# WGLab/DeepMod

Hardware: AMD Instinct MI355X
Metric: base-positions/sec (whole node), E. coli 5mC wd21/f7 BiLSTM (higher is better)
Workload: dtype f16x3

## Files before the change

### deepmod_amd/csrc/kern_f16q0.hip

```cpp
#include "kernels.h"
#include <utility>
#include "lstm_common.hip.inc"
#include "lstm_f16q.hip.inc"

static_assert(lstm16q::TILE_M == dmk::TILE_M, "work item size");

namespace {
inline void fill(lstmc::Params& p, const dmk::F16Args& a) {
    p.wpack = a.wpack;
    p.wpack_i8 = a.wpack;
    p.hpack = a.hpack;
    p.bout0 = p.bout1 = 0.0f;
    p.x = a.x;
    p.xstride = a.xstride;
    p.widx = a.widx;
    p.n = a.n;
    p.ntiles = a.ntiles;
    p.plogit = a.plogit;
    p.len_scale = std::ldexp(1.0f, -a.len_shift);
    p.len_mul = std::ldexp(1.0f, a.len_shift);
    p.range_flag = a.range_flag;
    for (int k = 0; k < 24; ++k) p.i8s[k] = a.i8s ? a.i8s[k] : 0.0f;
}
}
// ... 65 lines not shown
                                    d8[1] = (signed char)std::max(-127.0f, std::min(127.0f, ql));
                                }
                            }
                        }
                }
                for (int mrec = 0; mrec < (l == 0 ? 2 : 1); ++mrec) {
                    _Float16* dst = reinterpret_cast<_Float16*>(P.w.data() + off);
                    off += MIX_BYTES;
                    for (int rh = 0; rh < 2; ++rh)
                        for (int lane = 0; lane < 64; ++lane) {
                            const int m = lane & 15, g = lane >> 4;
                            const int unit = 8 * S + 4 * rh + m / 4, gate = m % 4;
                            _Float16 slot[8];
                            for (int j = 0; j < 8; ++j) slot[j] = (_Float16)0.0f;
                            if (unit < HID) {
                                const int gc = gate * 100 + unit;
                                _Float16 hi, lo;
                                if (mrec == 0) {
                                    split(wval(kin + 96 + g, gc, 1.0f), hi, lo);
                                    slot[0] = hi; slot[1] = lo; slot[2] = hi;
                                    split(wval(l == 0 ? g : 96 + g, gc, 1.0f), hi, lo);
                                    slot[3] = hi; slot[4] = lo; slot[5] = hi;
                                    if (g == 0) {
                                        split(wval(-2, gc, 1.0f), hi, lo);
                                        slot[6] = hi; slot[7] = lo;
                                    }
                                } else {
                                    split(g < 3 ? wval(4 + g, gc, 1.0f) : wval(NFEAT - 1, gc, len_mul), hi, lo);
                                    slot[0] = hi; slot[1] = lo; slot[2] = hi; slot[3] = lo;
                                }
                            }
                            for (int j = 0; j < 8; ++j) dst[(size_t(rh) * 64 + lane) * 8 + j] = slot[j];
                        }
                }
            }
        }
    }
    return P;
}


hipError_t f16q_prepare(int mm) {
    if (mm == 1) return f16q1_prepare();
    return hipFuncSetAttribute(reinterpret_cast<const void*>(lstm16q::bilstm_f16q_kernel<0>), hipFuncAttributeMaxDynamicSharedMemorySize, int(lstm16q::LDS_BYTES));
}
void f16q_launch(int mm, const F16Args& a, int grid, hipStream_t stream) {
    if (mm == 1) return f16q1_launch(a, grid, stream);
    lstmc::Params p;
    fill(p, a);
    hipLaunchKernelGGL(lstm16q::bilstm_f16q_kernel<0>, dim3(grid), dim3(lstm16q::THREADS), lstm16q::LDS_BYTES, stream, p);
}

}
```

### deepmod_amd/csrc/kern_f16q1.hip

```cpp
#include "kernels.h"
#include <utility>
#include "lstm_common.hip.inc"
#include "lstm_f16q.hip.inc"

namespace {
inline void fill(lstmc::Params& p, const dmk::F16Args& a) {
    p.wpack = a.wpack;
    p.wpack_i8 = a.wpack;
    p.hpack = a.hpack;
    p.bout0 = p.bout1 = 0.0f;
    p.x = a.x;
    p.xstride = a.xstride;
    p.widx = a.widx;
    p.n = a.n;
    p.ntiles = a.ntiles;
    p.plogit = a.plogit;
    p.len_scale = std::ldexp(1.0f, -a.len_shift);
    p.len_mul = std::ldexp(1.0f, a.len_shift);
    p.range_flag = a.range_flag;
    for (int k = 0; k < 24; ++k) p.i8s[k] = a.i8s ? a.i8s[k] : 0.0f;
}
}

namespace dmk {

hipError_t f16q1_prepare() {
    return hipFuncSetAttribute(reinterpret_cast<const void*>(lstm16q::bilstm_f16q_kernel<1>), hipFuncAttributeMaxDynamicSharedMemorySize, int(lstm16q::LDS_BYTES_I8));
}
void f16q1_launch(const F16Args& a, int grid, hipStream_t stream) {
    lstmc::Params p;
    fill(p, a);
    hipLaunchKernelGGL(lstm16q::bilstm_f16q_kernel<1>, dim3(grid), dim3(lstm16q::THREADS), lstm16q::LDS_BYTES_I8, stream, p);
}

}
```

### deepmod_amd/csrc/kernels.h

```cpp
#pragma once
#include <hip/hip_runtime.h>

#if defined(DM16Q_ABL_NOCELL) || defined(DM16Q_ABL_NODMA) || defined(DM16Q_ABL_MIX1) || defined(DM16Q_ABL_I8T) || defined(DM16Q_ABL_NOBAR) || defined(DM16Q_ABL_NOVMWAIT) || defined(DM16Q_AINIT) || defined(DM16Q_DEBUG_NOP) ||           \
    defined(DM16Q_NOCHUNK) || defined(DM16Q_NOPN) || defined(DM16Q_LOPACK) || defined(DM16Q_PRE) || defined(DM16Q_SNAKE) || defined(DM16Q_TRANS_COST) ||                     \
    defined(DM16S_ABL_2PROD) || defined(DM16S_ABL_B64) || defined(DM16S_ABL_LO_ONLY) || defined(DM16S_ABL_MFMA16) ||                              \
    defined(DM16S_ABL_MFMA16_PAD) || defined(DM16S_ABL_NOBAR) || defined(DM16S_ABL_NOCELL) || defined(DM16S_ABL_NODMA) ||                          \
    defined(DM16S_ABL_NOLDSA) || defined(DM16S_ADIST) || defined(DM16S_ALO_TRUNC) || defined(DM16S_PRE) || defined(DM_ABL_NOBAR) ||                \
    defined(DM_ABL_NODMA) || defined(DM_ABL_NOEPI) || defined(DM_ABL_NOSEQ) || defined(DM_TIMING) || defined(DM_TRACE) || defined(DM_TRACE2) ||   \
    defined(DM_WLO_TRUNC_ENV) || defined(DM_WLO_TRUNC_DEFAULT) || defined(DM_WITH_F16X3_ROLES) || defined(DM16R_DMA_M) ||                         \
    defined(DM_F16X3_SHAPE_DEFAULT) || defined(DM_WAVES) || defined(DM_MT) || defined(DM_WITH_F16S)
#define DM_ANY_EXPERIMENT_SWITCH 1
#ifndef DM_EXPERIMENT
#error "an ablation / experiment macro is defined without -DDM_EXPERIMENT: timing-only kernels must not be built into the product by a stray -D"
#endif
#else
#define DM_ANY_EXPERIMENT_SWITCH 0
#endif


#if defined(DM_WITH_F16X3_ROLES) && !defined(DM_WITH_F16S)
#error "the roles experiment lives in the translation unit of the 32x32x16 kernels: build it with -DDM_WITH_F16S as well"
#endif

#include <algorithm>
#include <cmath>
#include <cstdint>
#include <cstdlib>
#include <cstring>
#include <vector>

#include "../../include/deepmod_hip.h"

#ifndef DM_F16X3_SHAPE_DEFAULT
#define DM_F16X3_SHAPE_DEFAULT 16
#endif

namespace dmk {

constexpr int TILE_M = 128;

inline float gate_scale(int gc) { return (gc >= 100 && gc < 200) ? 2.8853900817779268f : -1.4426950408889634f; }


struct Packed32 {
    std::vector<float> w, b, h;
    float bout[2];
};

struct Packed16 {
    std::vector<unsigned char> w;
    float max_abs = 0.0f;
    bool finite = true;
    int len_shift = 0;
};

inline int choose_len_shift(const float* flat) {
    float m = 0.0f;
// ... 61 lines not shown
```

### deepmod_amd/csrc/lstm_f16q.hip.inc

```
#ifndef DM16Q_TRANS_COST
#define DM16Q_TRANS_COST 2
#endif
namespace lstm16q {

using lstmc::floatx2;
using lstmc::floatx4;
using lstmc::halfx2;
using lstmc::halfx8;
using lstmc::uintx4;
using lstmc::Params;
using lstmc::ex2;
using lstmc::rcp;
using lstmc::min60;
using lstmc::split_pack;
using lstmc::static_for;
using lstmc::as_h8;

constexpr int HID = 100, NFEAT = 7, WIN = 21, LIVE = 11;
constexpr int NTILE = 13;
constexpr int WAVES = 4, THREADS = 64 * WAVES, TILE_M = 32 * WAVES;
constexpr int KS_L0 = 4, KS_L12 = 7;
constexpr int REC_BYTES = 4096;
constexpr int MIX_BYTES = 2048;
constexpr int TILE_BYTES_L0 = (KS_L0 - 1) * REC_BYTES + 2 * MIX_BYTES, TILE_BYTES_L12 = (KS_L12 - 1) * REC_BYTES + MIX_BYTES;
constexpr int SLOT_BYTES = TILE_BYTES_L12;
constexpr int NSLOT = 2;
constexpr int C2_WAVE_BYTES = NTILE * 1024;
constexpr int C2_LAYER_BYTES = WAVES * C2_WAVE_BYTES;
constexpr size_t LDS_BYTES = size_t(NSLOT) * SLOT_BYTES + C2_LAYER_BYTES;
constexpr size_t LDS_BYTES_I8 = LDS_BYTES + C2_LAYER_BYTES;
constexpr size_t WEIGHT_BYTES_DIR = size_t(NTILE) * (TILE_BYTES_L0 + 2 * TILE_BYTES_L12);
constexpr size_t WEIGHT_BYTES = 2 * WEIGHT_BYTES_DIR;

using lstmc::intx4;
using lstmc::I8_MAGIC;
using lstmc::I8_HI_SCALE;
using lstmc::I8_LO_SCALE;
struct CellPipe {
    float ef[4], ei[4], ej[4], eo[4], t0[4], t1[4];
    unsigned hi01, hi23, lo01, lo23, i01, i23;
    floatx2 fold[2];
    floatx2 kmagic, khi, klo;
    static constexpr int NM = 14;
    template <int PRE, int FMT>
    __device__ static constexpr int nops(int M) {
        constexpr int n[9] = {12, 12, 12, 12, 8, 4, 4, 8, 6};
        if (M == 0) return PRE ? 16 : 0;
        if (M <= 9) return n[M - 1];
        if (M == 10) return FMT >= 1 ? 2 : 0;
        if (M == 11) return 4;
#if defined(DM16Q_LOPACK)
        if (M == 12) return FMT == 2 ? 2 : 0;
#else
        if (M == 12) return FMT != 1 ? 2 : 0;
#endif
        return FMT >= 1 ? 8 : 0;
    }
    template <int M, int J, int FMT = 0>
    __device__ __forceinline__ void op(floatx4 (&g)[4], const intx4 (&gi)[4], const floatx2 (&S)[2], float* c2, const bool only_a) {
        constexpr float K2 = 2.0f * 1.4426950408889634f;
        constexpr int q = J & 3, lv = J >> 2;
#define DM_PIN(X) asm volatile("" : "+v"(X))
        if constexpr (M == 0) {
            constexpr int k = J >> 1, c = k >> 1, pr = k & 1;
            if (only_a && (c & 1)) return;
            if constexpr ((J & 1) == 0) {
                fold[pr] = floatx2{(float)gi[c][2 * pr], (float)gi[c][2 * pr + 1]};
            } else {
                const floatx2 gp = __builtin_elementwise_fma(fold[pr], S[pr], floatx2{g[c][2 * pr], g[c][2 * pr + 1]});
                g[c][2 * pr] = gp[0];
                g[c][2 * pr + 1] = gp[1];
            }
            return;
        }
        if (only_a && (((M <= 8 || M == 11) && (q & 1)) || (M == 9 && lv == 0 && (q & 1)))) return;
        if constexpr (M == 1) {
            if constexpr (lv == 0) { t0[q] = min60(g[q][1]); DM_PIN(t0[q]); }
            else if constexpr (lv == 1) { ef[q] = ex2(g[q][2]); DM_PIN(ef[q]); }
            else { ei[q] = ex2(g[q][0]); DM_PIN(ei[q]); }
        } else if constexpr (M == 2) {
            if constexpr (lv == 0) { ej[q] = ex2(t0[q]); DM_PIN(ej[q]); }
            else if constexpr (lv == 1) { eo[q] = ex2(g[q][3]); DM_PIN(eo[q]); }
            else { ef[q] = 1.0f + ef[q]; DM_PIN(ef[q]); }
// ... 156 lines not shown
            asm volatile("ds_read_b128 %0, %1 offset:%2" : "=v"(a.loA) : "v"(addr), "i"(OFF + MIX_BYTES));
            if constexpr (WITH_B) asm volatile("ds_read_b128 %0, %1 offset:%2" : "=v"(a.loB) : "v"(addr), "i"(OFF + MIX_BYTES + 1024));
        }
    }
}
__host__ __device__ constexpr int a_reads(bool with_b, int mixed) { return (mixed == 1 ? 1 : 2) * (with_b ? 2 : 1); }
template <int N>
__device__ __forceinline__ void wait_a(AQuad& a) {
    asm volatile("s_waitcnt lgkmcnt(%4)" : "+v"(a.hiA), "+v"(a.loA), "+v"(a.hiB), "+v"(a.loB) : "i"(N));
}

#define DM16Q_STR2(X) #X
#define DM16Q_STR(X) DM16Q_STR2(X)
#if defined(DM16Q_NOPN)
#define DM16Q_AFTER_MFMA "s_nop " DM16Q_STR(DM16Q_NOPN)
#elif defined(DM16Q_DEBUG_NOP)
#define DM16Q_AFTER_MFMA "s_nop 15\n\ts_nop 15"
#else
#define DM16Q_AFTER_MFMA ""
#endif
#ifndef DM16Q_PRE
#define DM16Q_PRE 2
#endif

template <int LAYER, bool FIRST>
struct StageKind {
    static constexpr bool L0 = LAYER == 0;
    static constexpr int KS_FULL = L0 ? KS_L0 : KS_L12;
    static constexpr int KS = FIRST ? KS_FULL - 3 : KS_FULL;
    static constexpr int TILE_BYTES = L0 ? TILE_BYTES_L0 : TILE_BYTES_L12;
    static constexpr int DMA_OFF = FIRST ? 3 * REC_BYTES : 0;
    static constexpr int DMA_BYTES = TILE_BYTES - DMA_OFF;
    static constexpr int rec_off(int i) { return (FIRST ? 3 + i : i) * REC_BYTES; }
    static constexpr int mixed(int i) { return i == KS - 1 ? (L0 ? 2 : 1) : 0; }
    static constexpr bool is_own(int i) { return !FIRST && i < 3; }
    static constexpr int opnd(int i) { return FIRST ? i : (i < 3 ? i : i - 3); }
};

constexpr int quad(int t, int hh, int part) { return (t * 2 + hh) * 2 + part; }

struct WaveState {
    uintx4 own[3][12];
    unsigned m12[3][2][2];
    uintx4 nxt[12];
    float c2reg[NTILE][4];
    float c1reg[NTILE][4];
    floatx4 acc[3][4];
    intx4 acci[3][4];
    floatx2 i8s[3][2];
    CellPipe cp;
    float xf[2][2];
    int slot;
};

template <int LAYER, int MM>
__device__ __forceinline__ void c2_load(WaveState& w, const unsigned c2lds, const int tile, float (&row)[4]) {
    if constexpr (LAYER == 2) {
#pragma unroll
        for (int q = 0; q < 4; ++q) row[q] = w.c2reg[tile][q];
    } else if constexpr (LAYER == 1 && MM == 0) {
#pragma unroll
        for (int q = 0; q < 4; ++q) row[q] = w.c1reg[tile][q];
    } else {
        floatx4 v;
        asm volatile("ds_read_b128 %0, %1 offset:%2" : "=v"(v) : "v"(c2lds), "i"(LAYER * C2_LAYER_BYTES));
#pragma unroll
        for (int q = 0; q < 4; ++q) row[q] = v[q];
    }
}
template <int LAYER, int MM>
__device__ __forceinline__ void c2_store(WaveState& w, const unsigned c2lds, const int tile, const float (&row)[4]) {
    if constexpr (LAYER == 2) {
#pragma unroll
        for (int q = 0; q < 4; ++q) w.c2reg[tile][q] = row[q];
    } else if constexpr (LAYER == 1 && MM == 0) {
#pragma unroll
        for (int q = 0; q < 4; ++q) w.c1reg[tile][q] = row[q];
    } else {
        asm volatile("ds_write_b128 %0, %1 offset:%2" :: "v"(c2lds), "v"(floatx4{row[0], row[1], row[2], row[3]}), "i"(LAYER * C2_LAYER_BYTES) : "memory");
    }
}

__device__ __forceinline__ unsigned lo_lo(unsigned a, unsigned b) { return __builtin_amdgcn_perm(b, a, 0x05040100u); }
__device__ __forceinline__ unsigned hi_lo(unsigned a, unsigned b) { return __builtin_amdgcn_alignbit(b, a, 16); }

template <int LAYER, bool FIRST, int MM>
__device__ __forceinline__ void run_stage(const Params& p, WaveState& w, const unsigned lds_base, const unsigned c2_wave, const unsigned char* wdir, const int dir, const int s,
                                          const float* xwin0, const float* xwin1, const int wave_s, const unsigned lane16, const int grp, const unsigned one2) {
    using K = StageKind<LAYER, FIRST>;
    constexpr bool L0 = K::L0;
    constexpr int KS = K::KS;
    constexpr int PREV = (LAYER + 2) % 3;
    constexpr int I8 = (MM == 1 && !(L0 && FIRST)) ? 1 : 0;
    constexpr int PRE = I8;
    constexpr int PPRE = (MM == 1 && !(PREV == 0 && FIRST)) ? 1 : 0;
    constexpr int FMT = MM == 0 ? 0 : (LAYER == 2 ? 2 : 1);
    constexpr size_t LAYER_OFF[3] = {0, size_t(NTILE) * TILE_BYTES_L0, size_t(NTILE) * (TILE_BYTES_L0 + TILE_BYTES_L12)};
    uintx4 (&own)[12] = w.own[LAYER];
    const uintx4 (&inp)[12] = w.own[L0 ? 0 : LAYER - 1];
    const floatx2 (&S)[2] = w.i8s[LAYER];
    const floatx2 (&PS)[2] = w.i8s[PREV];
    uintx4 mx[2], mx2[2];
    unsigned x0p[2] = {0u, 0u}, x1a[2] = {0u, 0u}, x1b[2] = {0u, 0u};
    if constexpr (L0) {
        bool bad = false;
#pragma unroll
        for (int hh = 0; hh < 2; ++hh) {
            float v0 = w.xf[hh][0], v1 = w.xf[hh][1];
            bad |= !(fabsf(v0) <= 65504.0f);
            if (grp < 2) bad |= !(fabsf(v1) <= 65504.0f);
            else {
                const float t = rintf(v1 * p.len_scale);
                bad |= !(fabsf(t) <= 65504.0f);
                v1 = grp == 2 ? v1 - t * p.len_mul : t;
            }
            unsigned xh, xl;
            split_pack(v0, v1, xh, xl);
            x0p[hh] = lo_lo(xh, xl);
            x1a[hh] = __builtin_amdgcn_perm(xh, xh, 0x03020302u);
            x1b[hh] = __builtin_amdgcn_perm(xl, xl, 0x03020302u);
        }
        if (bad) *p.range_flag = 1;
        if (s + 1 < LIVE) {
            const int row = dir == 0 ? s + 1 : WIN - 2 - s;
            const int f1 = 4 + grp < NFEAT ? 4 + grp : NFEAT - 1;
            w.xf[0][0] = xwin0[row * NFEAT + grp]; w.xf[0][1] = xwin0[row * NFEAT + f1];
            w.xf[1][0] = xwin1[row * NFEAT + grp]; w.xf[1][1] = xwin1[row * NFEAT + f1];
        }
    }
    const bool last_stage = LAYER == 2 && s == LIVE - 1;
    static_for<NTILE>([&](auto Tc) {
        constexpr int T = decltype(Tc)::value;
        constexpr int P = T == 0 ? NTILE - 1 : T - 1;
        constexpr int accT = T == NTILE - 1 ? 2 : (T & 1), accP = P == NTILE - 1 ? 2 : (P & 1);
        constexpr bool WITH_B = T < NTILE - 1;
        constexpr int NMF = (WITH_B ? 4 : 2) * (I8 ? 2 : 3);
        float c2row[4];
        if constexpr (T == 0) c2_load<PREV, MM>(w, c2_wave + unsigned(NTILE - 1) * 1024u, NTILE - 1, c2row);
        else c2_load<LAYER, MM>(w, c2_wave + unsigned(P) * 1024u, P, c2row);
        const unsigned a_addr = lds_base + unsigned(w.slot) * SLOT_BYTES + lane16;
#ifdef DM16Q_AINIT
        AQuad a[2] = {};
#else
        AQuad a[2];
#endif
        load_a<K::rec_off(0), WITH_B, K::mixed(0)>(a[0], a_addr);
        if (!(last_stage && T == NTILE - 1)) {
            if constexpr (T + 1 < NTILE) {
                unsigned toff = unsigned(T + 1) * K::TILE_BYTES;
                asm volatile("" : "+s"(toff));
                stage_tile<K::DMA_BYTES>(wdir + (LAYER_OFF[LAYER] + K::DMA_OFF) + toff, lds_base + unsigned(w.slot ^ 1) * SLOT_BYTES + K::DMA_OFF, wave_s, lane16);
            } else {
                using KN = StageKind<(LAYER + 1) % 3, FIRST && LAYER < 2>;
                stage_tile<KN::DMA_BYTES>(wdir + (LAYER_OFF[(LAYER + 1) % 3] + KN::DMA_OFF), lds_base + unsigned(w.slot ^ 1) * SLOT_BYTES + KN::DMA_OFF, wave_s, lane16);
            }
        }
        floatx4 (&d)[4] = w.acc[accT];
        intx4 (&di)[4] = w.acci[accT];
        floatx4 (&g)[4] = w.acc[accP];
        const intx4 (&gi)[4] = w.acci[accP];
        const floatx4 z4 = {0.f, 0.f, 0.f, 0.f};
        const intx4 zi4 = {0, 0, 0, 0};
        constexpr int NCH = DM16Q_PRE + NMF * (KS - 1);
#ifdef DM16Q_NOCHUNK
#define DM_CHUNK(C) do { if constexpr ((C) == NCH - 1) { if constexpr (T == 0) w.cp.template all<PPRE, 0>(g, gi, PS, c2row, true); else w.cp.template all<PRE, FMT>(g, gi, S, c2row, false); } } while (0)
#else
#define DM_CHUNK(C) do { if constexpr (T == 0) w.cp.template chunk<(C), NCH, PPRE, 0>(g, gi, PS, c2row, true); else w.cp.template chunk<(C), NCH, PRE, FMT>(g, gi, S, c2row, false); } while (0)
#endif
        if constexpr (KS > 1) static_for<DM16Q_PRE>([&](auto cc) { DM_CHUNK(decltype(cc)::value); });
        static_for<KS>([&](auto ic) {
            constexpr int i = decltype(ic)::value;
            constexpr int MIXED = K::mixed(i);
            if constexpr (i + 1 < KS) load_a<K::rec_off(i + 1), WITH_B, K::mixed(i + 1)>(a[(i + 1) & 1], a_addr);
            if constexpr (i == KS - 1) {
                if constexpr (KS == 1) {
                    if constexpr (T == 0) w.cp.template all<PPRE, 0>(g, gi, PS, c2row, true);
                    else w.cp.template all<PRE, FMT>(g, gi, S, c2row, false);
                }
#ifdef DM16Q_ABL_NOCELL
                w.cp.hi01 = w.cp.hi23 = 0x2E662E66u; w.cp.lo01 = w.cp.lo23 = 0x0A660A66u;
#endif
                if constexpr (T == 0) {
                    w.m12[PREV][0][0] = lo_lo(w.cp.hi01, w.cp.hi01); w.m12[PREV][0][1] = lo_lo(w.cp.hi01, w.cp.lo01);
                    w.m12[PREV][1][0] = lo_lo(w.cp.hi23, w.cp.hi23); w.m12[PREV][1][1] = lo_lo(w.cp.hi23, w.cp.lo23);
                    c2_store<PREV, MM>(w, c2_wave + unsigned(NTILE - 1) * 1024u, NTILE - 1, c2row);
                } else {
                    constexpr int pt = P >> 2, pr = P & 3;
                    unsigned s01, s23;
                    if constexpr (FMT == 0) { s01 = w.cp.lo01; s23 = w.cp.lo23; }
                    else if constexpr (FMT == 1) { s01 = w.cp.i01; s23 = w.cp.i23; }
                    else { s01 = last_stage ? w.cp.lo01 : w.cp.i01; s23 = last_stage ? w.cp.lo23 : w.cp.i23; }
                    w.nxt[quad(pt, 0, 0)][pr] = w.cp.hi01; w.nxt[quad(pt, 0, 1)][pr] = s01;
                    w.nxt[quad(pt, 1, 0)][pr] = w.cp.hi23; w.nxt[quad(pt, 1, 1)][pr] = s23;
                    c2_store<LAYER, MM>(w, c2_wave + unsigned(P) * 1024u, P, c2row);
                }
            }
            if constexpr (T == 0) {
                static_for<3>([&](auto pc) {
                    constexpr int pt = decltype(pc)::value;
                    if constexpr (KS > 3 ? pt == i : i == 0) {
#pragma unroll
                        for (int e = 0; e < 4; ++e) w.own[PREV][4 * pt + e] = w.nxt[4 * pt + e];
                    }
                });
            }
            if constexpr (MIXED != 0 && T == 0) {
#pragma unroll
                for (int hh = 0; hh < 2; ++hh) {
                    unsigned in_hl;
                    if constexpr (L0) in_hl = x0p[hh];
                    else in_hl = w.m12[LAYER - 1][hh][1];
                    unsigned own_hh = w.m12[LAYER][hh][0], own_hl = w.m12[LAYER][hh][1];
                    asm volatile("" : "+v"(own_hh), "+v"(own_hl), "+v"(in_hl));
                    mx[hh] = uintx4{own_hh, hi_lo(own_hl, in_hl), in_hl, one2};
                    if constexpr (L0) mx2[hh] = uintx4{x1a[hh], x1b[hh], 0u, 0u};
                }
            }
            wait_a<(i + 1 < KS ? a_reads(WITH_B, K::mixed(i + 1 < KS ? i + 1 : i)) : 0)>(a[i & 1]);
            constexpr int C0 = DM16Q_PRE + NMF * i;
#define DM_MF(AOP, BOP, Q, NO)                                                                                              \
            d[Q] = __builtin_amdgcn_mfma_f32_16x16x32_f16(AOP, BOP, (i == 0 && (NO) == 0) ? z4 : d[Q], 0, 0, 0);              \
            asm volatile(DM16Q_AFTER_MFMA : "+v"(d[Q]) : "v"(AOP), "v"(BOP));
#define DM_MI(AOP, BOP, Q)                                                                                                  \
            di[Q] = __builtin_amdgcn_mfma_i32_16x16x64_i8(__builtin_bit_cast(intx4, AOP), __builtin_bit_cast(intx4, BOP), i == 0 ? zi4 : di[Q], 0, 0, 0); \
            asm volatile(DM16Q_AFTER_MFMA : "+v"(di[Q]) : "v"(AOP), "v"(BOP));
#define DM_CELLQ(N_) if constexpr (KS > 1 && i < KS - 1) DM_CHUNK(C0 + (N_))
            if constexpr (MIXED != 0) {
                const halfx8 b0 = as_h8(mx[0]), b1 = as_h8(mx[1]);
                DM_MF(a[i & 1].hiA, b0, 0, 0)
                DM_MF(a[i & 1].hiA, b1, 2, 0)
                if constexpr (WITH_B) { DM_MF(a[i & 1].hiB, b0, 1, 0) DM_MF(a[i & 1].hiB, b1, 3, 0) }
                if constexpr (MIXED == 2) {
                    const halfx8 e0 = as_h8(mx2[0]), e1 = as_h8(mx2[1]);
                    DM_MF(a[i & 1].loA, e0, 0, 1)
                    DM_MF(a[i & 1].loA, e1, 2, 1)
                    if constexpr (WITH_B) { DM_MF(a[i & 1].loB, e0, 1, 1) DM_MF(a[i & 1].loB, e1, 3, 1) }
                }
            } else {
                constexpr int t = K::opnd(i);
                halfx8 bh[2], bl[2];
#pragma unroll
                for (int hh = 0; hh < 2; ++hh) {
                    if constexpr (K::is_own(i)) { bh[hh] = as_h8(own[quad(t, hh, 0)]); bl[hh] = as_h8(own[quad(t, hh, 1)]); }
                    else { bh[hh] = as_h8(inp[quad(t, hh, 0)]); bl[hh] = as_h8(inp[quad(t, hh, 1)]); }
                }
                if constexpr (I8) {
                    DM_MF(a[i & 1].hiA, bh[0], 0, 0) DM_CELLQ(0);
                    DM_MF(a[i & 1].hiA, bh[1], 2, 0) DM_CELLQ(1);
                    if constexpr (WITH_B) { DM_MF(a[i & 1].hiB, bh[0], 1, 0) DM_CELLQ(2); DM_MF(a[i & 1].hiB, bh[1], 3, 0) DM_CELLQ(3); }
                    DM_MI(a[i & 1].loA, bl[0], 0) DM_CELLQ(WITH_B ? 4 : 2);
                    DM_MI(a[i & 1].loA, bl[1], 2) DM_CELLQ(WITH_B ? 5 : 3);
                    if constexpr (WITH_B) { DM_MI(a[i & 1].loB, bl[0], 1) DM_CELLQ(6); DM_MI(a[i & 1].loB, bl[1], 3) DM_CELLQ(7); }
                } else {
#ifdef DM16Q_SNAKE
                DM_MF(a[i & 1].hiA, bh[0], 0, 0) DM_CELLQ(0);
                if constexpr (WITH_B) { DM_MF(a[i & 1].hiB, bh[0], 1, 0) DM_CELLQ(1); DM_MF(a[i & 1].hiB, bh[1], 3, 0) DM_CELLQ(2); }
                DM_MF(a[i & 1].hiA, bh[1], 2, 0) DM_CELLQ(WITH_B ? 3 : 1);
                DM_MF(a[i & 1].loA, bh[1], 2, 1) DM_CELLQ(WITH_B ? 4 : 2);
                if constexpr (WITH_B) { DM_MF(a[i & 1].loB, bh[1], 3, 1) DM_CELLQ(5); DM_MF(a[i & 1].loB, bh[0], 1, 1) DM_CELLQ(6); }
                DM_MF(a[i & 1].loA, bh[0], 0, 1) DM_CELLQ(WITH_B ? 7 : 3);
                DM_MF(a[i & 1].hiA, bl[0], 0, 2) DM_CELLQ(WITH_B ? 8 : 4);
                if constexpr (WITH_B) { DM_MF(a[i & 1].hiB, bl[0], 1, 2) DM_CELLQ(9); DM_MF(a[i & 1].hiB, bl[1], 3, 2) DM_CELLQ(10); }
                DM_MF(a[i & 1].hiA, bl[1], 2, 2) DM_CELLQ(WITH_B ? 11 : 5);
#else
                DM_MF(a[i & 1].hiA, bh[0], 0, 0) DM_CELLQ(0);
                DM_MF(a[i & 1].hiA, bh[1], 2, 0) DM_CELLQ(1);
                if constexpr (WITH_B) { DM_MF(a[i & 1].hiB, bh[0], 1, 0) DM_CELLQ(2); DM_MF(a[i & 1].hiB, bh[1], 3, 0) DM_CELLQ(3); }
#ifdef DM16Q_ABL_I8T
                DM_MI(a[i & 1].loA, bl[0], 0) DM_CELLQ(WITH_B ? 4 : 2); DM_CELLQ(WITH_B ? 5 : 3);
                DM_MI(a[i & 1].loA, bl[1], 2) DM_CELLQ(WITH_B ? 6 : 4); DM_CELLQ(WITH_B ? 7 : 5);
                if constexpr (WITH_B) { DM_MI(a[i & 1].loB, bl[0], 1) DM_CELLQ(8); DM_CELLQ(9); DM_MI(a[i & 1].loB, bl[1], 3) DM_CELLQ(10); DM_CELLQ(11); }
#else
                DM_MF(a[i & 1].loA, bh[0], 0, 1) DM_CELLQ(WITH_B ? 4 : 2);
                DM_MF(a[i & 1].loA, bh[1], 2, 1) DM_CELLQ(WITH_B ? 5 : 3);
                if constexpr (WITH_B) { DM_MF(a[i & 1].loB, bh[0], 1, 1) DM_CELLQ(6); DM_MF(a[i & 1].loB, bh[1], 3, 1) DM_CELLQ(7); }
                DM_MF(a[i & 1].hiA, bl[0], 0, 2) DM_CELLQ(WITH_B ? 8 : 4);
                DM_MF(a[i & 1].hiA, bl[1], 2, 2) DM_CELLQ(WITH_B ? 9 : 5);
                if constexpr (WITH_B) { DM_MF(a[i & 1].hiB, bl[0], 1, 2) DM_CELLQ(10); DM_MF(a[i & 1].hiB, bl[1], 3, 2) DM_CELLQ(11); }
#endif
#endif
                }
            }
#undef DM_MF
#undef DM_MI
#undef DM_CELLQ
        });
#undef DM_CHUNK
#ifndef DM16Q_ABL_NOVMWAIT
        asm volatile("s_waitcnt vmcnt(0)" ::: "memory");
#endif
#ifndef DM16Q_ABL_NOBAR
        __builtin_amdgcn_s_barrier();
#endif
        w.slot ^= 1;
    });
}

template <int MM>
__global__ __launch_bounds__(THREADS, 1) void bilstm_f16q_kernel(const Params p) {
    extern __shared__ __attribute__((aligned(16))) unsigned char lds16q[];
    const int lane = threadIdx.x & 63;
    const int wave = threadIdx.x >> 6;
    const int wave_s = __builtin_amdgcn_readfirstlane(wave);
    const int grp = lane >> 4, n16 = lane & 15;
    const unsigned lane16 = unsigned(lane) * 16u;
    const unsigned lds_base = (unsigned)(size_t)lds16q;
    const unsigned c2_wave = lds_base + unsigned(NSLOT) * SLOT_BYTES + unsigned(wave) * C2_WAVE_BYTES + lane16;
    const unsigned one2 = grp == 0 ? 0x3C003C00u : 0u;
    const int nwork = 2 * p.ntiles;
    for (int work = blockIdx.x; work < nwork; work += gridDim.x) {
        const int tile = work >> 1, dir = work & 1;
        const long long tile0 = (long long)tile * TILE_M;
        const long long w_out = tile0 + wave * 32 + n16;
        long long wi0 = w_out, wi1 = w_out + 16;
        if (wi0 > p.n - 1) wi0 = p.n - 1;
        if (wi1 > p.n - 1) wi1 = p.n - 1;
        const float* xwin0 = p.x + (p.widx ? (long long)p.widx[wi0] : wi0) * p.xstride;
        const float* xwin1 = p.x + (p.widx ? (long long)p.widx[wi1] : wi1) * p.xstride;
        const unsigned char* wdir = p.wpack + size_t(dir) * WEIGHT_BYTES_DIR;

        WaveState w;
#pragma unroll
        for (int l = 0; l < 3; ++l) {
#pragma unroll
            for (int q = 0; q < 12; ++q) w.own[l][q] = uintx4{0u, 0u, 0u, 0u};
#pragma unroll
            for (int hh = 0; hh < 2; ++hh) w.m12[l][hh][0] = w.m12[l][hh][1] = 0u;
        }
#pragma unroll
        for (int q = 0; q < 12; ++q) w.nxt[q] = uintx4{0u, 0u, 0u, 0u};
#pragma unroll
        for (int t = 0; t < NTILE; ++t)
#pragma unroll
            for (int q = 0; q < 4; ++q) w.c2reg[t][q] = w.c1reg[t][q] = 0.0f;
#pragma unroll
        for (int t = 0; t < 3; ++t)
#pragma unroll
            for (int q = 0; q < 4; ++q) w.acc[t][q] = floatx4{0.f, 0.f, 0.f, 0.f};
        w.cp.hi01 = w.cp.hi23 = w.cp.lo01 = w.cp.lo23 = 0u;
        if constexpr (MM == 1) {
#pragma unroll
            for (int t = 0; t < 3; ++t)
#pragma unroll
                for (int q = 0; q < 4; ++q) w.acci[t][q] = intx4{0, 0, 0, 0};
#pragma unroll
            for (int l = 0; l < 3; ++l)
#pragma unroll
                for (int k = 0; k < 2; ++k) w.i8s[l][k] = floatx2{p.i8s[(dir * 3 + l) * 4 + 2 * k], p.i8s[(dir * 3 + l) * 4 + 2 * k + 1]};
            w.cp.kmagic = floatx2{I8_MAGIC, I8_MAGIC};
            w.cp.khi = floatx2{I8_HI_SCALE, I8_HI_SCALE};
            w.cp.klo = floatx2{I8_LO_SCALE, I8_LO_SCALE};
            w.cp.i01 = w.cp.i23 = 0u;
        }
        w.slot = 0;
        __syncthreads();
        {
            const floatx4 z4 = {0.f, 0.f, 0.f, 0.f};
#pragma unroll
            for (int t = 0; t < NTILE; ++t) {
                asm volatile("ds_write_b128 %0, %1" :: "v"(c2_wave + unsigned(t * 1024)), "v"(z4) : "memory");
                if constexpr (MM == 1) asm volatile("ds_write_b128 %0, %1 offset:%2" :: "v"(c2_wave + unsigned(t * 1024)), "v"(z4), "i"(C2_LAYER_BYTES) : "memory");
            }
        }
        {
            using K0 = StageKind<0, true>;
            stage_tile<K0::DMA_BYTES>(wdir + K0::DMA_OFF, lds_base + K0::DMA_OFF, wave_s, lane16);
        }
        {
            const int row = dir == 0 ? 0 : WIN - 1;
            const int f1 = 4 + grp < NFEAT ? 4 + grp : NFEAT - 1;
            w.xf[0][0] = xwin0[row * NFEAT + grp]; w.xf[0][1] = xwin0[row * NFEAT + f1];
            w.xf[1][0] = xwin1[row * NFEAT + grp]; w.xf[1][1] = xwin1[row * NFEAT + f1];
        }
        asm volatile("s_waitcnt vmcnt(0) lgkmcnt(0)" ::: "memory");
        __syncthreads();

#define DM_STAGE(LAYER, FIRST, S_) run_stage<LAYER, FIRST, MM>(p, w, lds_base, c2_wave, wdir, dir, S_, xwin0, xwin1, wave_s, lane16, grp, one2)
        DM_STAGE(0, true, 0);
        DM_STAGE(1, true, 0);
        DM_STAGE(2, true, 0);
        for (int s = 1; s < LIVE; ++s) {
            DM_STAGE(0, false, s);
            DM_STAGE(1, false, s);
            DM_STAGE(2, false, s);
        }
#undef DM_STAGE
        {
            float c2row[4];
#pragma unroll
            for (int q = 0; q < 4; ++q) c2row[q] = w.c2reg[NTILE - 1][q];
            w.cp.template all<MM, 0>(w.acc[2], w.acci[2], w.i8s[2], c2row, true);
            w.m12[2][0][1] = lo_lo(w.cp.hi01, w.cp.lo01);
            w.m12[2][1][1] = lo_lo(w.cp.hi23, w.cp.lo23);
#pragma unroll
            for (int q = 0; q < 12; ++q) w.own[2][q] = w.nxt[q];
        }
#pragma unroll
        for (int hh = 0; hh < 2; ++hh) {
            float hsum0 = 0.0f, hsum1 = 0.0f;
            static_for<NTILE>([&](auto Sc) {
                constexpr int S = decltype(Sc)::value;
                unsigned hi, lo;
                if constexpr (S < 12) { hi = w.own[2][quad(S >> 2, hh, 0)][S & 3]; lo = w.own[2][quad(S >> 2, hh, 1)][S & 3]; }
                else { hi = w.m12[2][hh][1]; lo = w.m12[2][hh][1] >> 16; }
                const halfx2 h2 = __builtin_bit_cast(halfx2, hi), l2 = __builtin_bit_cast(halfx2, lo);
#pragma unroll
                for (int rh = 0; rh < (S < 12 ? 2 : 1); ++rh) {
                    const float h = (float)h2[rh] + (float)l2[rh];
                    const float* wo = p.hpack + (dir * HID + 8 * S + 4 * rh + grp) * 2;
                    hsum0 = fmaf(h, wo[0], hsum0);
                    hsum1 = fmaf(h, wo[1], hsum1);
                }
            });
            hsum0 += __shfl_xor(hsum0, 16, 64);
            hsum1 += __shfl_xor(hsum1, 16, 64);
            hsum0 += __shfl_xor(hsum0, 32, 64);
            hsum1 += __shfl_xor(hsum1, 32, 64);
            if (lane < 16) {
                float* pl = p.plogit + (size_t(dir) * p.ntiles * TILE_M + size_t(w_out + 16 * hh)) * 2;
                pl[0] = hsum0;
                pl[1] = hsum1;
            }
        }
    }
}

}
```

Baseline: 48.06 million.

## Prefetch next work item's weights and inputs across item boundaries, cache head weights in LDS

The persistent kernel now prefetches the next work item's layer-0 weight tile and first input row during the last stage of the current item. This removes the per-item barrier, synchronous DMA and full wait at each item boundary. The output head weights are staged once into LDS, and the head dot product over the first tiles starts before the final cell update. KS==1 stages now interleave cell chunks with MFMAs, and optional timestamp probes are added under a macro. The risk is LDS slot reuse across items without a barrier, plus a larger LDS footprint.

```diff
diff --git a/deepmod_amd/csrc/kern_f16q0.hip b/deepmod_amd/csrc/kern_f16q0.hip
--- a/deepmod_amd/csrc/kern_f16q0.hip
+++ b/deepmod_amd/csrc/kern_f16q0.hip
@@ -141,3 +141,12 @@
 }
 
 }
+
+#ifdef DM16Q_STAMPS
+extern "C" int dm_f16q0_boundary_stamps(unsigned long long* out, int cap) {
+    const int n = lstm16q::STAMP_ITEMS * lstm16q::NSTAMP;
+    if (!out || cap < n) return 0;
+    if (hipMemcpyFromSymbol(out, HIP_SYMBOL(lstm16q::boundary_stamps), size_t(n) * sizeof(unsigned long long)) != hipSuccess) return -1;
+    return n;
+}
+#endif
diff --git a/deepmod_amd/csrc/kern_f16q1.hip b/deepmod_amd/csrc/kern_f16q1.hip
--- a/deepmod_amd/csrc/kern_f16q1.hip
+++ b/deepmod_amd/csrc/kern_f16q1.hip
@@ -34,3 +34,12 @@
 }
 
 }
+
+#ifdef DM16Q_STAMPS
+extern "C" int dm_f16q1_boundary_stamps(unsigned long long* out, int cap) {
+    const int n = lstm16q::STAMP_ITEMS * lstm16q::NSTAMP;
+    if (!out || cap < n) return 0;
+    if (hipMemcpyFromSymbol(out, HIP_SYMBOL(lstm16q::boundary_stamps), size_t(n) * sizeof(unsigned long long)) != hipSuccess) return -1;
+    return n;
+}
+#endif
diff --git a/deepmod_amd/csrc/kernels.h b/deepmod_amd/csrc/kernels.h
--- a/deepmod_amd/csrc/kernels.h
+++ b/deepmod_amd/csrc/kernels.h
@@ -2,7 +2,7 @@
 #include <hip/hip_runtime.h>
 
 #if defined(DM16Q_ABL_NOCELL) || defined(DM16Q_ABL_NODMA) || defined(DM16Q_ABL_MIX1) || defined(DM16Q_ABL_I8T) || defined(DM16Q_ABL_NOBAR) || defined(DM16Q_ABL_NOVMWAIT) || defined(DM16Q_AINIT) || defined(DM16Q_DEBUG_NOP) ||           \
-    defined(DM16Q_NOCHUNK) || defined(DM16Q_NOPN) || defined(DM16Q_LOPACK) || defined(DM16Q_PRE) || defined(DM16Q_SNAKE) || defined(DM16Q_TRANS_COST) ||                     \
+    defined(DM16Q_NOCHUNK) || defined(DM16Q_NOPN) || defined(DM16Q_LOPACK) || defined(DM16Q_PRE) || defined(DM16Q_SNAKE) || defined(DM16Q_TRANS_COST) || defined(DM16Q_STAMPS) ||                     \
     defined(DM16S_ABL_2PROD) || defined(DM16S_ABL_B64) || defined(DM16S_ABL_LO_ONLY) || defined(DM16S_ABL_MFMA16) ||                              \
     defined(DM16S_ABL_MFMA16_PAD) || defined(DM16S_ABL_NOBAR) || defined(DM16S_ABL_NOCELL) || defined(DM16S_ABL_NODMA) ||                          \
     defined(DM16S_ABL_NOLDSA) || defined(DM16S_ADIST) || defined(DM16S_ALO_TRUNC) || defined(DM16S_PRE) || defined(DM_ABL_NOBAR) ||                \
diff --git a/deepmod_amd/csrc/lstm_f16q.hip.inc b/deepmod_amd/csrc/lstm_f16q.hip.inc
--- a/deepmod_amd/csrc/lstm_f16q.hip.inc
+++ b/deepmod_amd/csrc/lstm_f16q.hip.inc
@@ -27,8 +27,10 @@
 constexpr int NSLOT = 2;
 constexpr int C2_WAVE_BYTES = NTILE * 1024;
 constexpr int C2_LAYER_BYTES = WAVES * C2_WAVE_BYTES;
-constexpr size_t LDS_BYTES = size_t(NSLOT) * SLOT_BYTES + C2_LAYER_BYTES;
+constexpr int HEAD_BYTES = 2 * HID * 2 * 4;
+constexpr size_t LDS_BYTES = size_t(NSLOT) * SLOT_BYTES + C2_LAYER_BYTES + HEAD_BYTES;
 constexpr size_t LDS_BYTES_I8 = LDS_BYTES + C2_LAYER_BYTES;
+template <int MM> constexpr unsigned HEAD_OFF = unsigned(NSLOT) * SLOT_BYTES + unsigned(MM == 1 ? 2 : 1) * C2_LAYER_BYTES;
 constexpr size_t WEIGHT_BYTES_DIR = size_t(NTILE) * (TILE_BYTES_L0 + 2 * TILE_BYTES_L12);
 constexpr size_t WEIGHT_BYTES = 2 * WEIGHT_BYTES_DIR;
 
@@ -291,6 +293,10 @@
     float xf[2][2];
     int slot;
 };
+struct NextItem {
+    int work;
+    const float *x0, *x1;
+};
 
 template <int LAYER, int MM>
 __device__ __forceinline__ void c2_load(WaveState& w, const unsigned c2lds, const int tile, float (&row)[4]) {
@@ -325,7 +331,7 @@
 
 template <int LAYER, bool FIRST, int MM>
 __device__ __forceinline__ void run_stage(const Params& p, WaveState& w, const unsigned lds_base, const unsigned c2_wave, const unsigned char* wdir, const int dir, const int s,
-                                          const float* xwin0, const float* xwin1, const int wave_s, const unsigned lane16, const int grp, const unsigned one2) {
+                                          const float* xwin0, const float* xwin1, const NextItem& nx, const int wave_s, const unsigned lane16, const int grp, const unsigned one2) {
     using K = StageKind<LAYER, FIRST>;
     constexpr bool L0 = K::L0;
     constexpr int KS = K::KS;
@@ -360,11 +366,14 @@
             x1b[hh] = __builtin_amdgcn_perm(xl, xl, 0x03020302u);
         }
         if (bad) *p.range_flag = 1;
+        const int f1 = 4 + grp < NFEAT ? 4 + grp : NFEAT - 1;
         if (s + 1 < LIVE) {
             const int row = dir == 0 ? s + 1 : WIN - 2 - s;
-            const int f1 = 4 + grp < NFEAT ? 4 + grp : NFEAT - 1;
             w.xf[0][0] = xwin0[row * NFEAT + grp]; w.xf[0][1] = xwin0[row * NFEAT + f1];
             w.xf[1][0] = xwin1[row * NFEAT + grp]; w.xf[1][1] = xwin1[row * NFEAT + f1];
+        } else {
+            w.xf[0][0] = nx.x0[grp]; w.xf[0][1] = nx.x0[f1];
+            w.xf[1][0] = nx.x1[grp]; w.xf[1][1] = nx.x1[f1];
         }
     }
     const bool last_stage = LAYER == 2 && s == LIVE - 1;
@@ -384,15 +393,16 @@
         AQuad a[2];
 #endif
         load_a<K::rec_off(0), WITH_B, K::mixed(0)>(a[0], a_addr);
-        if (!(last_stage && T == NTILE - 1)) {
-            if constexpr (T + 1 < NTILE) {
-                unsigned toff = unsigned(T + 1) * K::TILE_BYTES;
-                asm volatile("" : "+s"(toff));
-                stage_tile<K::DMA_BYTES>(wdir + (LAYER_OFF[LAYER] + K::DMA_OFF) + toff, lds_base + unsigned(w.slot ^ 1) * SLOT_BYTES + K::DMA_OFF, wave_s, lane16);
-            } else {
-                using KN = StageKind<(LAYER + 1) % 3, FIRST && LAYER < 2>;
-                stage_tile<KN::DMA_BYTES>(wdir + (LAYER_OFF[(LAYER + 1) % 3] + KN::DMA_OFF), lds_base + unsigned(w.slot ^ 1) * SLOT_BYTES + KN::DMA_OFF, wave_s, lane16);
-            }
+        if constexpr (T + 1 < NTILE) {
+            unsigned toff = unsigned(T + 1) * K::TILE_BYTES;
+            asm volatile("" : "+s"(toff));
+            stage_tile<K::DMA_BYTES>(wdir + (LAYER_OFF[LAYER] + K::DMA_OFF) + toff, lds_base + unsigned(w.slot ^ 1) * SLOT_BYTES + K::DMA_OFF, wave_s, lane16);
+        } else if (last_stage) {
+            using K0 = StageKind<0, true>;
+            stage_tile<K0::DMA_BYTES>(p.wpack + size_t(nx.work & 1) * WEIGHT_BYTES_DIR + K0::DMA_OFF, lds_base + unsigned(w.slot ^ 1) * SLOT_BYTES + K0::DMA_OFF, wave_s, lane16);
+        } else {
+            using KN = StageKind<(LAYER + 1) % 3, FIRST && LAYER < 2>;
+            stage_tile<KN::DMA_BYTES>(wdir + (LAYER_OFF[(LAYER + 1) % 3] + KN::DMA_OFF), lds_base + unsigned(w.slot ^ 1) * SLOT_BYTES + KN::DMA_OFF, wave_s, lane16);
         }
         floatx4 (&d)[4] = w.acc[accT];
         intx4 (&di)[4] = w.acci[accT];
@@ -400,40 +410,38 @@
         const intx4 (&gi)[4] = w.acci[accP];
         const floatx4 z4 = {0.f, 0.f, 0.f, 0.f};
         const intx4 zi4 = {0, 0, 0, 0};
-        constexpr int NCH = DM16Q_PRE + NMF * (KS - 1);
+        static_assert(KS > 1 || L0, "a stage of one k32-step is layer 0 at step 0");
+        constexpr int NCH = KS > 1 ? DM16Q_PRE + NMF * (KS - 1) : DM16Q_PRE + (WITH_B ? 8 : 4);
 #ifdef DM16Q_NOCHUNK
 #define DM_CHUNK(C) do { if constexpr ((C) == NCH - 1) { if constexpr (T == 0) w.cp.template all<PPRE, 0>(g, gi, PS, c2row, true); else w.cp.template all<PRE, FMT>(g, gi, S, c2row, false); } } while (0)
 #else
 #define DM_CHUNK(C) do { if constexpr (T == 0) w.cp.template chunk<(C), NCH, PPRE, 0>(g, gi, PS, c2row, true); else w.cp.template chunk<(C), NCH, PRE, FMT>(g, gi, S, c2row, false); } while (0)
 #endif
-        if constexpr (KS > 1) static_for<DM16Q_PRE>([&](auto cc) { DM_CHUNK(decltype(cc)::value); });
+        static_for<DM16Q_PRE>([&](auto cc) { DM_CHUNK(decltype(cc)::value); });
+        auto cells_done = [&]() {
+#ifdef DM16Q_ABL_NOCELL
+            w.cp.hi01 = w.cp.hi23 = 0x2E662E66u; w.cp.lo01 = w.cp.lo23 = 0x0A660A66u;
+#endif
+            if constexpr (T == 0) {
+                w.m12[PREV][0][0] = lo_lo(w.cp.hi01, w.cp.hi01); w.m12[PREV][0][1] = lo_lo(w.cp.hi01, w.cp.lo01);
+                w.m12[PREV][1][0] = lo_lo(w.cp.hi23, w.cp.hi23); w.m12[PREV][1][1] = lo_lo(w.cp.hi23, w.cp.lo23);
+                c2_store<PREV, MM>(w, c2_wave + unsigned(NTILE - 1) * 1024u, NTILE - 1, c2row);
+            } else {
+                constexpr int pt = P >> 2, pr = P & 3;
+                unsigned s01, s23;
+                if constexpr (FMT == 0) { s01 = w.cp.lo01; s23 = w.cp.lo23; }
+                else if constexpr (FMT == 1) { s01 = w.cp.i01; s23 = w.cp.i23; }
+                else { s01 = last_stage ? w.cp.lo01 : w.cp.i01; s23 = last_stage ? w.cp.lo23 : w.cp.i23; }
+                w.nxt[quad(pt, 0, 0)][pr] = w.cp.hi01; w.nxt[quad(pt, 0, 1)][pr] = s01;
+                w.nxt[quad(pt, 1, 0)][pr] = w.cp.hi23; w.nxt[quad(pt, 1, 1)][pr] = s23;
+                c2_store<LAYER, MM>(w, c2_wave + unsigned(P) * 1024u, P, c2row);
+            }
+        };
         static_for<KS>([&](auto ic) {
             constexpr int i = decltype(ic)::value;
             constexpr int MIXED = K::mixed(i);
             if constexpr (i + 1 < KS) load_a<K::rec_off(i + 1), WITH_B, K::mixed(i + 1)>(a[(i + 1) & 1], a_addr);
-            if constexpr (i == KS - 1) {
-                if constexpr (KS == 1) {
-                    if constexpr (T == 0) w.cp.template all<PPRE, 0>(g, gi, PS, c2row, true);
-                    else w.cp.template all<PRE, FMT>(g, gi, S, c2row, false);
-                }
-#ifdef DM16Q_ABL_NOCELL
-                w.cp.hi01 = w.cp.hi23 = 0x2E662E66u; w.cp.lo01 = w.cp.lo23 = 0x0A660A66u;
-#endif
-                if constexpr (T == 0) {
-                    w.m12[PREV][0][0] = lo_lo(w.cp.hi01, w.cp.hi01); w.m12[PREV][0][1] = lo_lo(w.cp.hi01, w.cp.lo01);
-                    w.m12[PREV][1][0] = lo_lo(w.cp.hi23, w.cp.hi23); w.m12[PREV][1][1] = lo_lo(w.cp.hi23, w.cp.lo23);
-                    c2_store<PREV, MM>(w, c2_wave + unsigned(NTILE - 1) * 1024u, NTILE - 1, c2row);
-                } else {
-                    constexpr int pt = P >> 2, pr = P & 3;
-                    unsigned s01, s23;
-                    if constexpr (FMT == 0) { s01 = w.cp.lo01; s23 = w.cp.lo23; }
-                    else if constexpr (FMT == 1) { s01 = w.cp.i01; s23 = w.cp.i23; }
-                    else { s01 = last_stage ? w.cp.lo01 : w.cp.i01; s23 = last_stage ? w.cp.lo23 : w.cp.i23; }
-                    w.nxt[quad(pt, 0, 0)][pr] = w.cp.hi01; w.nxt[quad(pt, 0, 1)][pr] = s01;
-                    w.nxt[quad(pt, 1, 0)][pr] = w.cp.hi23; w.nxt[quad(pt, 1, 1)][pr] = s23;
-                    c2_store<LAYER, MM>(w, c2_wave + unsigned(P) * 1024u, P, c2row);
-                }
-            }
+            if constexpr (i == KS - 1 && KS > 1) cells_done();
             if constexpr (T == 0) {
                 static_for<3>([&](auto pc) {
                     constexpr int pt = decltype(pc)::value;
@@ -464,17 +472,19 @@
             di[Q] = __builtin_amdgcn_mfma_i32_16x16x64_i8(__builtin_bit_cast(intx4, AOP), __builtin_bit_cast(intx4, BOP), i == 0 ? zi4 : di[Q], 0, 0, 0); \
             asm volatile(DM16Q_AFTER_MFMA : "+v"(di[Q]) : "v"(AOP), "v"(BOP));
 #define DM_CELLQ(N_) if constexpr (KS > 1 && i < KS - 1) DM_CHUNK(C0 + (N_))
+#define DM_CELL1(N_) if constexpr (KS == 1) DM_CHUNK(DM16Q_PRE + (N_))
             if constexpr (MIXED != 0) {
                 const halfx8 b0 = as_h8(mx[0]), b1 = as_h8(mx[1]);
-                DM_MF(a[i & 1].hiA, b0, 0, 0)
-                DM_MF(a[i & 1].hiA, b1, 2, 0)
-                if constexpr (WITH_B) { DM_MF(a[i & 1].hiB, b0, 1, 0) DM_MF(a[i & 1].hiB, b1, 3, 0) }
+                DM_MF(a[i & 1].hiA, b0, 0, 0) DM_CELL1(0);
+                DM_MF(a[i & 1].hiA, b1, 2, 0) DM_CELL1(1);
+                if constexpr (WITH_B) { DM_MF(a[i & 1].hiB, b0, 1, 0) DM_CELL1(2); DM_MF(a[i & 1].hiB, b1, 3, 0) DM_CELL1(3); }
                 if constexpr (MIXED == 2) {
                     const halfx8 e0 = as_h8(mx2[0]), e1 = as_h8(mx2[1]);
-                    DM_MF(a[i & 1].loA, e0, 0, 1)
-                    DM_MF(a[i & 1].loA, e1, 2, 1)
-                    if constexpr (WITH_B) { DM_MF(a[i & 1].loB, e0, 1, 1) DM_MF(a[i & 1].loB, e1, 3, 1) }
+                    DM_MF(a[i & 1].loA, e0, 0, 1) DM_CELL1(WITH_B ? 4 : 2);
+                    DM_MF(a[i & 1].loA, e1, 2, 1) DM_CELL1(WITH_B ? 5 : 3);
+                    if constexpr (WITH_B) { DM_MF(a[i & 1].loB, e0, 1, 1) DM_CELL1(6); DM_MF(a[i & 1].loB, e1, 3, 1) DM_CELL1(7); }
                 }
+                if constexpr (KS == 1) cells_done();
             } else {
                 constexpr int t = K::opnd(i);
                 halfx8 bh[2], bl[2];
@@ -523,6 +533,7 @@
 #undef DM_MF
 #undef DM_MI
 #undef DM_CELLQ
+#undef DM_CELL1
         });
 #undef DM_CHUNK
 #ifndef DM16Q_ABL_NOVMWAIT
@@ -534,6 +545,14 @@
         w.slot ^= 1;
     });
 }
+
+#ifdef DM16Q_STAMPS
+constexpr int STAMP_ITEMS = 4096, NSTAMP = 8;
+static __device__ unsigned long long boundary_stamps[STAMP_ITEMS * NSTAMP];
+#define DM_STAMP(K_) do { if (threadIdx.x == 0 && work < STAMP_ITEMS) boundary_stamps[work * NSTAMP + (K_)] = __builtin_amdgcn_s_memtime(); } while (0)
+#else
+#define DM_STAMP(K_) do { } while (0)
+#endif
 
 template <int MM>
 __global__ __launch_bounds__(THREADS, 1) void bilstm_f16q_kernel(const Params p) {
@@ -547,18 +566,33 @@
     const unsigned c2_wave = lds_base + unsigned(NSLOT) * SLOT_BYTES + unsigned(wave) * C2_WAVE_BYTES + lane16;
     const unsigned one2 = grp == 0 ? 0x3C003C00u : 0u;
     const int nwork = 2 * p.ntiles;
+    WaveState w;
     for (int work = blockIdx.x; work < nwork; work += gridDim.x) {
+        DM_STAMP(0);
         const int tile = work >> 1, dir = work & 1;
         const long long tile0 = (long long)tile * TILE_M;
         const long long w_out = tile0 + wave * 32 + n16;
         long long wi0 = w_out, wi1 = w_out + 16;
         if (wi0 > p.n - 1) wi0 = p.n - 1;
         if (wi1 > p.n - 1) wi1 = p.n - 1;
-        const float* xwin0 = p.x + (p.widx ? (long long)p.widx[wi0] : wi0) * p.xstride;
-        const float* xwin1 = p.x + (p.widx ? (long long)p.widx[wi1] : wi1) * p.xstride;
+        NextItem nx;
+        nx.work = work + int(gridDim.x) < nwork ? work + int(gridDim.x) : work;
+        long long ni0 = (long long)(nx.work >> 1) * TILE_M + wave * 32 + n16, ni1 = ni0 + 16;
+        if (ni0 > p.n - 1) ni0 = p.n - 1;
+        if (ni1 > p.n - 1) ni1 = p.n - 1;
+        if (p.widx) {
+            const int i0 = p.widx[wi0], i1 = p.widx[wi1], j0 = p.widx[ni0], j1 = p.widx[ni1];
+            wi0 = i0; wi1 = i1; ni0 = j0; ni1 = j1;
+        }
+        const float* xwin0 = p.x + wi0 * p.xstride;
+        const float* xwin1 = p.x + wi1 * p.xstride;
         const unsigned char* wdir = p.wpack + size_t(dir) * WEIGHT_BYTES_DIR;
-
-        WaveState w;
+        {
+            const int row = (nx.work & 1) == 0 ? 0 : WIN - 1;
+            nx.x0 = p.x + ni0 * p.xstride + row * NFEAT;
+            nx.x1 = p.x + ni1 * p.xstride + row * NFEAT;
+        }
+
 #pragma unroll
         for (int l = 0; l < 3; ++l) {
 #pragma unroll
@@ -591,8 +625,6 @@
             w.cp.klo = floatx2{I8_LO_SCALE, I8_LO_SCALE};
             w.cp.i01 = w.cp.i23 = 0u;
         }
-        w.slot = 0;
-        __syncthreads();
         {
             const floatx4 z4 = {0.f, 0.f, 0.f, 0.f};
 #pragma unroll
@@ -601,67 +633,95 @@
                 if constexpr (MM == 1) asm volatile("ds_write_b128 %0, %1 offset:%2" :: "v"(c2_wave + unsigned(t * 1024)), "v"(z4), "i"(C2_LAYER_BYTES) : "memory");
             }
         }
-        {
-            using K0 = StageKind<0, true>;
-            stage_tile<K0::DMA_BYTES>(wdir + K0::DMA_OFF, lds_base + K0::DMA_OFF, wave_s, lane16);
-        }
-        {
-            const int row = dir == 0 ? 0 : WIN - 1;
-            const int f1 = 4 + grp < NFEAT ? 4 + grp : NFEAT - 1;
-            w.xf[0][0] = xwin0[row * NFEAT + grp]; w.xf[0][1] = xwin0[row * NFEAT + f1];
-            w.xf[1][0] = xwin1[row * NFEAT + grp]; w.xf[1][1] = xwin1[row * NFEAT + f1];
-        }
-        asm volatile("s_waitcnt vmcnt(0) lgkmcnt(0)" ::: "memory");
-        __syncthreads();
-
-#define DM_STAGE(LAYER, FIRST, S_) run_stage<LAYER, FIRST, MM>(p, w, lds_base, c2_wave, wdir, dir, S_, xwin0, xwin1, wave_s, lane16, grp, one2)
+        if (work == int(blockIdx.x)) {
+            w.slot = 0;
+            {
+                float* hw = reinterpret_cast<float*>(lds16q + HEAD_OFF<MM>);
+                for (int i = threadIdx.x; i < HEAD_BYTES / 4; i += THREADS) hw[i] = p.hpack[i];
+            }
+            {
+                using K0 = StageKind<0, true>;
+                stage_tile<K0::DMA_BYTES>(wdir + K0::DMA_OFF, lds_base + K0::DMA_OFF, wave_s, lane16);
+            }
+            {
+                const int row = dir == 0 ? 0 : WIN - 1;
+                const int f1 = 4 + grp < NFEAT ? 4 + grp : NFEAT - 1;
+                w.xf[0][0] = xwin0[row * NFEAT + grp]; w.xf[0][1] = xwin0[row * NFEAT + f1];
+                w.xf[1][0] = xwin1[row * NFEAT + grp]; w.xf[1][1] = xwin1[row * NFEAT + f1];
+            }
+            asm volatile("s_waitcnt vmcnt(0) lgkmcnt(0)" ::: "memory");
+            __syncthreads();
+        }
+        DM_STAMP(1);
+
+#define DM_STAGE(LAYER, FIRST, S_) run_stage<LAYER, FIRST, MM>(p, w, lds_base, c2_wave, wdir, dir, S_, xwin0, xwin1, nx, wave_s, lane16, grp, one2)
         DM_STAGE(0, true, 0);
+        DM_STAMP(2);
         DM_STAGE(1, true, 0);
+        DM_STAMP(3);
         DM_STAGE(2, true, 0);
+        DM_STAMP(4);
         for (int s = 1; s < LIVE; ++s) {
             DM_STAGE(0, false, s);
             DM_STAGE(1, false, s);
             DM_STAGE(2, false, s);
+#ifdef DM16Q_STAMPS
+            if (s == 1) DM_STAMP(5);
+#endif
         }
 #undef DM_STAGE
+        DM_STAMP(6);
+        float hsum[2][2] = {{0.0f, 0.0f}, {0.0f, 0.0f}};
+        const floatx2* hw = reinterpret_cast<const floatx2*>(lds16q + HEAD_OFF<MM>) + (dir * HID + grp);
+        static_for<NTILE - 1>([&](auto Sc) {
+            constexpr int S = decltype(Sc)::value;
+#pragma unroll
+            for (int rh = 0; rh < 2; ++rh) {
+                const floatx2 wo = hw[8 * S + 4 * rh];
+#pragma unroll
+                for (int hh = 0; hh < 2; ++hh) {
+                    const unsigned hi = w.nxt[quad(S >> 2, hh, 0)][S & 3], lo = w.nxt[quad(S >> 2, hh, 1)][S & 3];
+                    const halfx2 h2 = __builtin_bit_cast(halfx2, hi), l2 = __builtin_bit_cast(halfx2, lo);
+                    const float h = (float)h2[rh] + (float)l2[rh];
+                    hsum[hh][0] = fmaf(h, wo[0], hsum[hh][0]);
+                    hsum[hh][1] = fmaf(h, wo[1], hsum[hh][1]);
+                }
+            }
+        });
         {
             float c2row[4];
 #pragma unroll
             for (int q = 0; q < 4; ++q) c2row[q] = w.c2reg[NTILE - 1][q];
             w.cp.template all<MM, 0>(w.acc[2], w.acci[2], w.i8s[2], c2row, true);
-            w.m12[2][0][1] = lo_lo(w.cp.hi01, w.cp.lo01);
-            w.m12[2][1][1] = lo_lo(w.cp.hi23, w.cp.lo23);
-#pragma unroll
-            for (int q = 0; q < 12; ++q) w.own[2][q] = w.nxt[q];
+            const floatx2 wo = hw[8 * (NTILE - 1)];
+            const unsigned m[2] = {lo_lo(w.cp.hi01, w.cp.lo01), lo_lo(w.cp.hi23, w.cp.lo23)};
+#pragma unroll
+            for (int hh = 0; hh < 2; ++hh) {
+                const halfx2 h2 = __builtin_bit_cast(halfx2, m[hh]), l2 = __builtin_bit_cast(halfx2, m[hh] >> 16);
+                const float h = (float)h2[0] + (float)l2[0];
+                hsum[hh][0] = fmaf(h, wo[0], hsum[hh][0]);
+                hsum[hh][1] = fmaf(h, wo[1], hsum[hh][1]);
+            }
         }
 #pragma unroll
         for (int hh = 0; hh < 2; ++hh) {
-            float hsum0 = 0.0f, hsum1 = 0.0f;
-            static_for<NTILE>([&](auto Sc) {
-                constexpr int S = decltype(Sc)::value;
-                unsigned hi, lo;
-                if constexpr (S < 12) { hi = w.own[2][quad(S >> 2, hh, 0)][S & 3]; lo = w.own[2][quad(S >> 2, hh, 1)][S & 3]; }
-                else { hi = w.m12[2][hh][1]; lo = w.m12[2][hh][1] >> 16; }
-                const halfx2 h2 = __builtin_bit_cast(halfx2, hi), l2 = __builtin_bit_cast(halfx2, lo);
-#pragma unroll
-                for (int rh = 0; rh < (S < 12 ? 2 : 1); ++rh) {
-                    const float h = (float)h2[rh] + (float)l2[rh];
-                    const float* wo = p.hpack + (dir * HID + 8 * S + 4 * rh + grp) * 2;
-                    hsum0 = fmaf(h, wo[0], hsum0);
-                    hsum1 = fmaf(h, wo[1], hsum1);
-                }
-            });
-            hsum0 += __shfl_xor(hsum0, 16, 64);
-            hsum1 += __shfl_xor(hsum1, 16, 64);
-            hsum0 += __shfl_xor(hsum0, 32, 64);
-            hsum1 += __shfl_xor(hsum1, 32, 64);
-            if (lane < 16) {
+#pragma unroll
+            for (int c = 0; c < 2; ++c) {
+                hsum[hh][c] += __shfl_xor(hsum[hh][c], 16, 64);
+                hsum[hh][c] += __shfl_xor(hsum[hh][c], 32, 64);
+            }
+        }
+        if (lane < 16) {
+#pragma unroll
+            for (int hh = 0; hh < 2; ++hh) {
                 float* pl = p.plogit + (size_t(dir) * p.ntiles * TILE_M + size_t(w_out + 16 * hh)) * 2;
-                pl[0] = hsum0;
-                pl[1] = hsum1;
-            }
-        }
+                pl[0] = hsum[hh][0];
+                pl[1] = hsum[hh][1];
+            }
+        }
+        DM_STAMP(7);
     }
 }
+#undef DM_STAMP
 
 }
```

Measured after the change: 48.51 million (median of 6 runs). No clear change (+0.9%).
